# vkit-dev/vkit-ocr-model-adaptive-scaling

Measured on AMD Instinct MI355X. Metric: images/sec fwd+bwd @1024x1024 bf16 (train step: rough+precise passes, losses, backward, clip, AdamW), higher is better.
Workload: dtype bf16

## Files before the change

### include/vkas.h

```cpp
#ifndef VKAS_H
#define VKAS_H

#include <stddef.h>
#include <stdint.h>

#ifdef __cplusplus
extern "C" {
#endif

#define VKAS_F32 0
#define VKAS_BF16 1
#define VKAS_F16 2

#define VKAS_OK 0
#define VKAS_E_ARG (-1)
#define VKAS_E_LAUNCH (-2)

#define VKAS_EPI_NONE 0
#define VKAS_EPI_GELU 1
#define VKAS_EPI_SCALE_RES 2
#define VKAS_EPI_DGELU 3
#define VKAS_EPI_ADD 4
#define VKAS_EPI_PATCH 5
#define VKAS_EPI_HEAD 6
// ... 42 lines not shown
long vkas_layernorm_bwd_parts(long M, int Cp);
long vkas_scale_res_bwd_parts(long M, int Cp);
long vkas_dwconv7x7_wgrad_parts(int B, int H, int W, int Cp, int dtype);
int vkas_pad_vector(const float* v, float* out, int n, int np, void* stream);
size_t vkas_dw_weight_elems(int Cp);
int vkas_pack_dw_weight(const float* w, float* out, int C, int Cp, int flip, void* stream);
int vkas_unpack_dw_wgrad(const float* gw, float* grad, int C, int Cp, int accumulate, void* stream);
int vkas_image_nchw_to_nhwc8(const float* img, void* out, int B, int C, int H, int W, int dtype, void* stream);
int vkas_nhwc_to_nchw_f32(const void* x, long ld, float* out, int B, int H, int W, int C, int dtype, void* stream);
int vkas_nchw_f32_to_nhwc(const float* g, void* out, long ld, int B, int H, int W, int C, int Cp, int dtype, void* stream);

int vkas_conv_gemm_fwd(const void* x, const vkas_conv_geom* g, const void* Bw, int Np, const vkas_epilogue* epi,
                       int dtype, void* stream);
int vkas_conv_gemm_wgrad(const void* x, const vkas_conv_geom* g, const void* dy, long lddy, int Np, float* gw,
                         float* gb, int dtype, void* stream);
int vkas_conv_gemm_wgrad_ordered(const void* x, const vkas_conv_geom* g, const void* dy, long lddy, int Np, float* gw,
                                 int dtype, void* stream);
int vkas_conv_gemm_wgrad_gelu(const void* x, const vkas_conv_geom* g, const void* dy, long lddy, int Np, float* gw,
                              float* gb, int dtype, void* stream);

size_t vkas_upconv5_fold_elems(int Np, int Cp, int f, int transposed);
int vkas_upconv5_fold(const float* w, void* out, int N, int C, int Np, int Cp, int f, int transposed, int dtype, void* stream);
int vkas_upconv5_fwd(const void* x, const vkas_conv_geom* g, int f, const void* Bf, int Np, const float* bias, void* out,
                     long ldo, int dtype, void* stream);
int vkas_upconv5_dgrad(const void* dy, long lddy, const vkas_conv_geom* g, int f, const void* Bt, int Np, void* dx, long lddx,
                       int dtype, void* stream);
size_t vkas_upconv5_wgrad_ws_bytes(int B, int H, int W, int Np);
int vkas_upconv5_wgrad(const void* x, const vkas_conv_geom* g, int f, const void* dy, long lddy, int Np, void* ws,
                       size_t ws_bytes, float* gwf, float* gb, int dtype, void* stream);
int vkas_upconv5_unfold_wgrad(const float* gwf, float* dw, int N, int C, int Np, int Cp, int f, int accumulate, void* stream);

size_t vkas_mlp_chain_image_elems(int C);
int vkas_mlp_chain_pack(const float* w1, const float* w2, const float* b1, int C, int mode, void* img, int dtype,
                        void* stream);
int vkas_mlp_chain_fwd(const void* yn, long ldyn, const void* img, const float* b2, const void* x, long ldx,
                       const float* colscale, const float* rowscale, int rows_per_image, void* h, long ldh, void* z,
                       long ldz, void* out, long ldo, long M, int C, int dtype, void* stream);
int vkas_mlp_chain_ln_fwd(const void* y, long ldy, const float* ln_gamma, const float* ln_beta, void* yn, long ldyn,
                          float* stats, const void* img, const float* b2, const void* x, long ldx, const float* colscale,
                          const float* rowscale, int rows_per_image, void* h, long ldh, void* z, long ldz, void* out,
                          long ldo, long M, int C, int dtype, void* stream);
int vkas_mlp_chain_bwd(const void* dz, long lddz, const void* img_t, const void* h, long ldh, void* dh, long lddh,
                       void* dyn, long lddyn, long M, int C, int dtype, void* stream);
int vkas_conv_gemm_tile(int wgrad, long M, int Np, int K);
int vkas_conv_gemm_kernel_id(int wgrad, const vkas_conv_geom* g, int Np, long lddy, int head_width);
int vkas_colsum(const void* y, long ld, long M, int Np, float* out, int accumulate, float* ws, size_t ws_bytes,
                int dtype, void* stream);
size_t vkas_colsum_ws_bytes(long M, int Np);

int vkas_dwconv7x7_fwd(const void* x, long ldx, const float* w, const float* bias, const void* addend, long ldadd,
                       void* y, long ldy, int B, int H, int W, int Cp, int dtype, void* stream);
int vkas_dwconv7x7_wgrad(const void* x, long ldx, const void* dy, long lddy, float* gw, float* gb, float* ws,
                         size_t ws_bytes, int B, int H, int W, int Cp, int dtype, void* stream);
size_t vkas_dwconv7x7_wgrad_ws_bytes(int B, int H, int W, int Cp);

int vkas_layernorm_fwd(const void* x, long ldx, const float* gamma, const float* beta, void* y, long ldy,
                       float* stats, long M, int C, int Cp, int act_gelu, int dtype, void* stream);
int vkas_layernorm_bwd(const void* x, long ldx, const float* gamma, const float* beta, const float* stats,
                       const void* dy, long lddy, void* dx, long lddx, float* dgamma, float* dbeta, float* ws,
                       size_t ws_bytes, long M, int C, int Cp, int act_gelu, int dtype, void* stream);
size_t vkas_layernorm_bwd_ws_bytes(long M, int Cp);

int vkas_pack_head_params(const float* gamma, const float* beta, const float* wproj, const float* bproj, int C, int oc,
                          int pw, float* out, void* stream);
int vkas_head_tail_fwd(const void* z, long ldz, const vkas_head_desc* hd, long M, int dtype, void* stream);
int vkas_head_tail_bwd(const void* z, long ldz, const vkas_head_desc* hd, const float* const* dproj, void* dz, long lddz,
                       float* dparams, float* ws, size_t ws_bytes, long M, int dtype, void* stream);
size_t vkas_head_tail_bwd_ws_bytes(long M, int pw);

int vkas_scale_res_bwd(const void* dout, long lddo, const void* z, long ldz, const float* colscale,
                       const float* rowscale, int rows_per_image, void* dz, long lddz, float* dscale, float* dbias,
                       float* ws, size_t ws_bytes, long M, int Cp, int dtype, void* stream);
size_t vkas_scale_res_bwd_ws_bytes(long M, int Cp);

int vkas_resize_fwd(const void* x, long ldx, void* y, long ldy, int B, int Hin, int Win, int Hout, int Wout,
                    int Cp, int mode, int accumulate, int dtype, void* stream);
int vkas_resize_bwd(const void* dy, long lddy, void* dx, long lddx, int B, int Hin, int Win, int Hout, int Wout,
                    int Cp, int mode, int accumulate, int dtype, void* stream);
size_t vkas_resize_bwd_ws_bytes(int B, int Hin, int Win, int Hout, int Wout, int Cp);
int vkas_resize_bwd_ws(const void* dy, long lddy, void* dx, long lddx, float* ws, size_t ws_bytes, int B, int Hin, int Win,
                       int Hout, int Wout, int Cp, int mode, int accumulate, int dtype, void* stream);

int vkas_upconv_adj(const void* dz, long lddz, void* E, int B, int h, int w, int N, int dtype, void* stream);
int vkas_upconv_adj_unpack_wgrad(const float* gE, float* gwp, int N, int Cp, void* stream);

int vkas_adaptive_avgpool_fwd(const void* x, long ldx, void* y, long ldy, int B, int H, int W, int s, int Cp,
                              int dtype, void* stream);
int vkas_adaptive_avgpool_bwd(const void* dy, long lddy, void* dx, long lddx, int B, int H, int W, int s, int Cp,
                              int accumulate, int dtype, void* stream);

int vkas_copy_channels(const void* x, long ldx, void* y, long ldy, long M, int Cp, int accumulate, int dtype,
                       void* stream);
int vkas_copy_channel_range(const void* x, long ldx, int c_src, void* y, long ldy, int c_dst, long M, int C,
                            int zero_tail, int dtype, void* stream);
int vkas_softplus_fwd(const float* x, float* y, long n, void* stream);
int vkas_softplus_bwd(const float* x, const float* dy, float* dx, long n, void* stream);

typedef struct vkas_rough_loss_cfg {
  float focal_factor, dice_factor, l1_factor, score_min, height_min;
  float focal_alpha, focal_gamma;
  float out_scale;
} vkas_rough_loss_cfg;
int vkas_rough_loss_fwd(const float* mask_feat, const float* height_feat, const float* gt_mask,
                        const float* gt_score, int B, int H, int W, int up, int left, int CH, int CW,
                        const vkas_rough_loss_cfg* cfg, double* sums, float* loss, void* stream);
int vkas_rough_loss_bwd(const float* mask_feat, const float* height_feat, const float* gt_mask,
                        const float* gt_score, int B, int H, int W, int up, int left, int CH, int CW,
                        const vkas_rough_loss_cfg* cfg, const double* sums, const float* dloss, float* d_mask_feat,
                        float* d_height_feat, void* stream);

typedef struct vkas_precise_loss_cfg {
  float pos_l2, neg_l2, offset_l1, reg_l1, angle_ce, dist_l1, loss_factor;
  float smooth_beta;
  float out_scale;
} vkas_precise_loss_cfg;
int vkas_points_margin(const int64_t* py, const int64_t* px, long n, int H, int W, int64_t* margin, void* stream);
int vkas_precise_loss_fwd(const float* prob, const float* offset, const float* angle, const float* dist,
                          const float* gt_score, const float* gt_mask, const int64_t* py, const int64_t* px,
                          const float* gt_offsets, const float* gt_angles, const float* gt_dists, int B, int H,
                          int W, int up, int left, int CH, int CW, int P, const vkas_precise_loss_cfg* cfg,
                          double* sums, float* loss, void* stream);
int vkas_precise_loss_bwd(const float* prob, const float* offset, const float* angle, const float* dist,
                          const float* gt_score, const float* gt_mask, const int64_t* py, const int64_t* px,
                          const float* gt_offsets, const float* gt_angles, const float* gt_dists, int B, int H,
                          int W, int up, int left, int CH, int CW, int P, const vkas_precise_loss_cfg* cfg,
                          const double* sums, const float* dloss, float* d_prob, float* d_offset, float* d_angle,
                          float* d_dist, void* stream);
typedef struct vkas_precise_loss_extra_cfg {
  float mask_focal, prob_l1, prob_wahr;
  float prob_l1_beta;
  float wahr_gamma;
  float focal_alpha, focal_gamma;
} vkas_precise_loss_extra_cfg;
#define VKAS_PRECISE_LOSS_EX_SUMS 16
int vkas_precise_loss_ex_fwd(const float* prob, const float* offset, const float* angle, const float* dist,
                             const float* gt_score, const float* gt_mask, const int64_t* py, const int64_t* px,
                             const float* gt_offsets, const float* gt_angles, const float* gt_dists, int B, int H,
                             int W, int up, int left, int CH, int CW, int P, const vkas_precise_loss_cfg* cfg,
                             const float* mask_feat, const vkas_precise_loss_extra_cfg* ex, double* sums, float* loss,
                             void* stream);
int vkas_precise_loss_ex_bwd(const float* prob, const float* offset, const float* angle, const float* dist,
                             const float* gt_score, const float* gt_mask, const int64_t* py, const int64_t* px,
                             const float* gt_offsets, const float* gt_angles, const float* gt_dists, int B, int H,
                             int W, int up, int left, int CH, int CW, int P, const vkas_precise_loss_cfg* cfg,
                             const float* mask_feat, const vkas_precise_loss_extra_cfg* ex, const double* sums,
                             const float* dloss, float* d_prob, float* d_offset, float* d_angle, float* d_dist,
                             float* d_mask_feat, void* stream);

#define VKAS_LOSS_FOCAL 0
#define VKAS_LOSS_DICE 1
#define VKAS_LOSS_L1 2
#define VKAS_LOSS_SMOOTH_L1 3
#define VKAS_LOSS_L2 4
#define VKAS_LOSS_WAHR 5
int vkas_elementwise_loss_fwd(int kind, const float* pred, const float* gt, const float* mask, long n, float p0, float p1,
                              float eps, double* sums, float* loss, void* stream);
int vkas_elementwise_loss_bwd(int kind, const float* pred, const float* gt, const float* mask, long n, float p0, float p1,
                              float eps, const double* sums, const float* dloss, float* dpred, void* stream);
int vkas_cross_entropy_fwd(const float* logits, const void* target, int hard, long rows, int classes, double* sums,
                           float* loss, void* stream);
int vkas_cross_entropy_bwd(const float* logits, const void* target, int hard, long rows, int classes, const float* dloss,
                           float* dlogits, void* stream);

int vkas_points_prepare(const long* py, const long* px, int B, int P, int H, int W, int* map, int* pix, long Mp, void* stream);
int vkas_points_gather_rows(const void* z, long ldz, int c0, int Ns, const float* stats, const float* const* dproj,
                            int n_heads, long M, const int* pix, long Mp, void* zs, float* stats_s, float* dproj_s,
// ... 43 lines not shown
```

### vkit_ocr_model_adaptive_scaling_amd/_lib.py

```python
import ctypes
import os
from ctypes import POINTER, Structure, c_char_p, c_double, c_float, c_int, c_int64, c_long, c_longlong, c_size_t, c_void_p

_HERE = os.path.dirname(os.path.abspath(__file__))
LIB_PATH = os.environ.get('VKAS_LIB_PATH') or os.path.join(_HERE, 'libvkas.so')

F32, BF16, F16 = 0, 1, 2
EPI_NONE, EPI_GELU, EPI_SCALE_RES, EPI_DGELU, EPI_ADD, EPI_PATCH, EPI_HEAD = range(7)
LOSS_FOCAL, LOSS_DICE, LOSS_L1, LOSS_SMOOTH_L1, LOSS_L2 = range(5)
LOSS_WAHR = 5
PRECISE_LOSS_EX_SUMS = 16


class ConvGeom(Structure):
    _fields_ = [('B', c_int), ('Hin', c_int), ('Win', c_int), ('Hout', c_int), ('Wout', c_int), ('Cp', c_int),
                ('ldx', c_int), ('KH', c_int), ('KW', c_int), ('stride', c_int), ('pad', c_int)]


class HeadDesc(Structure):
    _fields_ = [('n_heads', c_int), ('pw', c_int), ('n0', c_int * 4), ('np', c_int * 4), ('c', c_int * 4),
                ('oc', c_int * 4), ('params', c_void_p), ('stats', c_void_p), ('proj', c_void_p)]


class Epilogue(Structure):
# ... 18 lines not shown
    _fields_ = [('pos_l2', c_float), ('neg_l2', c_float), ('offset_l1', c_float), ('reg_l1', c_float),
                ('angle_ce', c_float), ('dist_l1', c_float), ('loss_factor', c_float), ('smooth_beta', c_float),
                ('out_scale', c_float)]


class PreciseLossExtraCfg(Structure):
    _fields_ = [('mask_focal', c_float), ('prob_l1', c_float), ('prob_wahr', c_float), ('prob_l1_beta', c_float),
                ('wahr_gamma', c_float), ('focal_alpha', c_float), ('focal_gamma', c_float)]


class VkasError(RuntimeError):
    pass


if not os.path.exists(LIB_PATH):
    raise ImportError(
        f'{LIB_PATH} not found: build the HIP kernels first (python -c "import __graft_entry__ as g; g.build()" '
        f'or make -C {os.path.join(_HERE, "csrc")}).  There is no CPU fallback.')

lib = ctypes.CDLL(LIB_PATH)

_P = c_void_p
_SIGS = {
    'vkas_last_error': (c_char_p, []),
    'vkas_abi_version': (c_int, []),
    'vkas_pack_conv_weight': (c_int, [_P, _P, c_int, c_int, c_int, c_int, c_int, c_int, c_int, c_int, _P]),
    'vkas_pack_conv_weight_slice': (c_int, [_P, _P, c_int, c_int, c_int, c_int, c_int, c_int, c_int, c_int, c_int, c_int, _P]),
    'vkas_unpack_conv_wgrad': (c_int, [_P, _P, c_int, c_int, c_int, c_int, c_int, c_int, c_int, _P]),
    'vkas_accumulate_many': (c_int, [c_int, POINTER(c_void_p), POINTER(c_void_p), POINTER(c_int), _P]),
    'vkas_finalize_many': (c_int, [c_int, POINTER(c_void_p), POINTER(c_long), POINTER(c_int), POINTER(c_int), POINTER(c_void_p),
                                   POINTER(c_int), _P]),
    'vkas_layernorm_bwd_parts': (c_long, [c_long, c_int]),
    'vkas_scale_res_bwd_parts': (c_long, [c_long, c_int]),
    'vkas_dwconv7x7_wgrad_parts': (c_long, [c_int, c_int, c_int, c_int, c_int]),
    'vkas_pad_vector': (c_int, [_P, _P, c_int, c_int, _P]),
    'vkas_dw_weight_elems': (c_size_t, [c_int]),
    'vkas_pack_dw_weight': (c_int, [_P, _P, c_int, c_int, c_int, _P]),
    'vkas_unpack_dw_wgrad': (c_int, [_P, _P, c_int, c_int, c_int, _P]),
    'vkas_image_nchw_to_nhwc8': (c_int, [_P, _P, c_int, c_int, c_int, c_int, c_int, _P]),
    'vkas_nhwc_to_nchw_f32': (c_int, [_P, c_long, _P, c_int, c_int, c_int, c_int, c_int, _P]),
    'vkas_nchw_f32_to_nhwc': (c_int, [_P, _P, c_long, c_int, c_int, c_int, c_int, c_int, c_int, _P]),
    'vkas_conv_gemm_fwd': (c_int, [_P, POINTER(ConvGeom), _P, c_int, POINTER(Epilogue), c_int, _P]),
    'vkas_conv_gemm_wgrad': (c_int, [_P, POINTER(ConvGeom), _P, c_long, c_int, _P, _P, c_int, _P]),
    'vkas_conv_gemm_wgrad_ordered': (c_int, [_P, POINTER(ConvGeom), _P, c_long, c_int, _P, c_int, _P]),
    'vkas_conv_gemm_wgrad_gelu': (c_int, [_P, POINTER(ConvGeom), _P, c_long, c_int, _P, _P, c_int, _P]),
    'vkas_upconv5_fold_elems': (c_size_t, [c_int, c_int, c_int, c_int]),
    'vkas_upconv5_fold': (c_int, [_P, _P, c_int, c_int, c_int, c_int, c_int, c_int, c_int, _P]),
    'vkas_upconv5_fwd': (c_int, [_P, POINTER(ConvGeom), c_int, _P, c_int, _P, _P, c_long, c_int, _P]),
    'vkas_upconv5_dgrad': (c_int, [_P, c_long, POINTER(ConvGeom), c_int, _P, c_int, _P, c_long, c_int, _P]),
    'vkas_upconv5_wgrad_ws_bytes': (c_size_t, [c_int, c_int, c_int, c_int]),
    'vkas_upconv5_wgrad': (c_int, [_P, POINTER(ConvGeom), c_int, _P, c_long, c_int, _P, c_size_t, _P, _P, c_int, _P]),
    'vkas_upconv5_unfold_wgrad': (c_int, [_P, _P, c_int, c_int, c_int, c_int, c_int, c_int, _P]),
    'vkas_mlp_chain_image_elems': (c_size_t, [c_int]),
    'vkas_mlp_chain_pack': (c_int, [_P, _P, _P, c_int, c_int, _P, c_int, _P]),
    'vkas_mlp_chain_fwd': (c_int, [_P, c_long, _P, _P, _P, c_long, _P, _P, c_int, _P, c_long, _P, c_long, _P, c_long,
                                   c_long, c_int, c_int, _P]),
    'vkas_mlp_chain_ln_fwd': (c_int, [_P, c_long, _P, _P, _P, c_long, _P, _P, _P, _P, c_long, _P, _P, c_int, _P, c_long, _P,
                                      c_long, _P, c_long, c_long, c_int, c_int, _P]),
    'vkas_mlp_chain_bwd': (c_int, [_P, c_long, _P, _P, c_long, _P, c_long, _P, c_long, c_long, c_int, c_int, _P]),
    'vkas_conv_gemm_tile': (c_int, [c_int, c_long, c_int, c_int]),
    'vkas_conv_gemm_kernel_id': (c_int, [c_int, POINTER(ConvGeom), c_int, c_long, c_int]),
    'vkas_colsum': (c_int, [_P, c_long, c_long, c_int, _P, c_int, _P, c_size_t, c_int, _P]),
    'vkas_colsum_ws_bytes': (c_size_t, [c_long, c_int]),
    'vkas_dwconv7x7_fwd': (c_int, [_P, c_long, _P, _P, _P, c_long, _P, c_long, c_int, c_int, c_int, c_int, c_int, _P]),
    'vkas_dwconv7x7_wgrad': (c_int, [_P, c_long, _P, c_long, _P, _P, _P, c_size_t, c_int, c_int, c_int, c_int, c_int, _P]),
    'vkas_dwconv7x7_wgrad_ws_bytes': (c_size_t, [c_int, c_int, c_int, c_int]),
    'vkas_layernorm_fwd': (c_int, [_P, c_long, _P, _P, _P, c_long, _P, c_long, c_int, c_int, c_int, c_int, _P]),
    'vkas_layernorm_bwd': (c_int, [_P, c_long, _P, _P, _P, _P, c_long, _P, c_long, _P, _P, _P, c_size_t, c_long, c_int,
                                   c_int, c_int, c_int, _P]),
    'vkas_layernorm_bwd_ws_bytes': (c_size_t, [c_long, c_int]),
    'vkas_pack_head_params': (c_int, [_P, _P, _P, _P, c_int, c_int, c_int, _P, _P]),
    'vkas_head_tail_fwd': (c_int, [_P, c_long, _P, c_long, c_int, _P]),
    'vkas_head_tail_bwd': (c_int, [_P, c_long, POINTER(HeadDesc), POINTER(c_void_p), _P, c_long, _P, _P, c_size_t, c_long, c_int, _P]),
    'vkas_head_tail_bwd_ws_bytes': (c_size_t, [c_long, c_int]),
    'vkas_scale_res_bwd': (c_int, [_P, c_long, _P, c_long, _P, _P, c_int, _P, c_long, _P, _P, _P, c_size_t, c_long,
                                   c_int, c_int, _P]),
    'vkas_scale_res_bwd_ws_bytes': (c_size_t, [c_long, c_int]),
    'vkas_resize_fwd': (c_int, [_P, c_long, _P, c_long, c_int, c_int, c_int, c_int, c_int, c_int, c_int, c_int, c_int, _P]),
    'vkas_resize_bwd': (c_int, [_P, c_long, _P, c_long, c_int, c_int, c_int, c_int, c_int, c_int, c_int, c_int, c_int, _P]),
    'vkas_resize_bwd_ws_bytes': (c_size_t, [c_int, c_int, c_int, c_int, c_int, c_int]),
    'vkas_resize_bwd_ws': (c_int, [_P, c_long, _P, c_long, _P, c_size_t, c_int, c_int, c_int, c_int, c_int, c_int, c_int, c_int,
                                   c_int, _P]),
    'vkas_upconv_adj': (c_int, [_P, c_long, _P, c_int, c_int, c_int, c_int, c_int, _P]),
    'vkas_upconv_adj_unpack_wgrad': (c_int, [_P, _P, c_int, c_int, _P]),
    'vkas_adaptive_avgpool_fwd':(c_int, [_P, c_long, _P, c_long, c_int, c_int, c_int, c_int, c_int, c_int, _P]),
    'vkas_adaptive_avgpool_bwd': (c_int, [_P, c_long, _P, c_long, c_int, c_int, c_int, c_int, c_int, c_int, c_int, _P]),
    'vkas_copy_channels': (c_int, [_P, c_long, _P, c_long, c_long, c_int, c_int, c_int, _P]),
    'vkas_copy_channel_range': (c_int, [_P, c_long, c_int, _P, c_long, c_int, c_long, c_int, c_int, c_int, _P]),
    'vkas_softplus_fwd': (c_int, [_P, _P, c_long, _P]),
    'vkas_softplus_bwd': (c_int, [_P, _P, _P, c_long, _P]),
    'vkas_rough_loss_fwd': (c_int, [_P, _P, _P, _P, c_int, c_int, c_int, c_int, c_int, c_int, c_int,
                                    POINTER(RoughLossCfg), _P, _P, _P]),
    'vkas_rough_loss_bwd': (c_int, [_P, _P, _P, _P, c_int, c_int, c_int, c_int, c_int, c_int, c_int,
                                    POINTER(RoughLossCfg), _P, _P, _P, _P, _P]),
    'vkas_points_margin': (c_int, [_P, _P, c_long, c_int, c_int, _P, _P]),
    'vkas_precise_loss_fwd': (c_int, [_P] * 11 + [c_int] * 8 + [POINTER(PreciseLossCfg), _P, _P, _P]),
    'vkas_precise_loss_bwd': (c_int, [_P] * 11 + [c_int] * 8 + [POINTER(PreciseLossCfg), _P, _P, _P, _P, _P, _P, _P]),
    'vkas_precise_loss_ex_fwd': (c_int, [_P] * 11 + [c_int] * 8 + [POINTER(PreciseLossCfg), _P, POINTER(PreciseLossExtraCfg),
                                                                     _P, _P, _P]),
    'vkas_precise_loss_ex_bwd': (c_int, [_P] * 11 + [c_int] * 8 + [POINTER(PreciseLossCfg), _P, POINTER(PreciseLossExtraCfg)]
                                 + [_P] * 8),
    'vkas_elementwise_loss_fwd': (c_int, [c_int, _P, _P, _P, c_long, c_float, c_float, c_float, _P, _P, _P]),
    'vkas_elementwise_loss_bwd': (c_int, [c_int, _P, _P, _P, c_long, c_float, c_float, c_float, _P, _P, _P, _P]),
    'vkas_cross_entropy_fwd': (c_int, [_P, _P, c_int, c_long, c_int, _P, _P, _P]),
    'vkas_cross_entropy_bwd': (c_int, [_P, _P, c_int, c_long, c_int, _P, _P, _P]),
    'vkas_points_prepare': (c_int, [_P, _P, c_int, c_int, c_int, c_int, _P, _P, c_long, _P]),
    'vkas_points_gather_rows': (c_int, [_P, c_long, c_int, c_int, _P, _P, c_int, c_long, _P, c_long, _P, _P, _P, c_int, _P]),
    'vkas_points_gather_patches': (c_int, [_P, c_long, c_int, c_int, c_int, c_int, _P, c_long, _P, c_int, _P]),
    'vkas_points_scatter3x3': (c_int, [_P, _P, _P, c_long, c_int, c_int, c_int, c_int, _P, c_long, c_int, _P]),
    'vkas_points_scatter_vec8': (c_int, [_P, _P, c_long, _P, _P]),
    'vkas_points_gather_vec8': (c_int, [_P, _P, c_long, _P, _P]),
    'vkas_pack_many': (c_int, [_P, _P, c_int, c_int, _P]),
    'vkas_pack_many_blocks': (c_int, [_P]),
    'vkas_rough_postprocess': (c_int, [_P, _P, c_int, c_int, c_int, _P, _P, c_float, c_float, _P, _P, _P]),
    'vkas_precise_postprocess': (c_int, [_P, _P, _P, _P, c_int, c_int, c_int, _P, _P, _P, _P, _P, _P, _P]),
    'vkas_char_polygons_workspace_bytes': (c_long, [c_int, c_int, c_int, c_int]),
    'vkas_char_polygons': (c_int, [_P, _P, _P, _P, c_int, c_int, c_int, c_int, c_float, c_float, c_float, _P, c_size_t,
                                   _P, _P, _P, _P, _P]),
    'vkas_text_regions_workspace_bytes': (c_longlong, [c_int, c_int, c_int, c_int]),
    'vkas_text_regions': (c_int, [_P, _P, c_int, c_int, c_int, c_int, _P, c_longlong, _P, _P, _P, _P, _P, _P, _P]),
    'vkas_l2norm_sq': (c_int, [_P, c_long, _P, _P]),
    'vkas_adamw_step': (c_int, [_P, _P, _P, _P, c_long, _P, c_float, c_float, c_float, c_float, c_float, c_float,
                                c_float, c_int, _P]),
}

EXPORTS = tuple(_SIGS)

for _name, (_res, _args) in _SIGS.items():
    _fn = getattr(lib, _name)
    _fn.restype = _res
    _fn.argtypes = _args


def check(rc: int, what: str = ''):
    if rc != 0:
        msg = lib.vkas_last_error()
        raise VkasError(f'{what}: vkas error {rc}: {msg.decode() if msg else "?"}')
```

### vkit_ocr_model_adaptive_scaling_amd/csrc/upconv_adj.hip

```cpp
#include "vkas_common.h"

namespace {

__device__ __forceinline__ int xcd_row(unsigned bx, unsigned rows) {
  const unsigned xcd = bx & 7u, slot = bx >> 3;
  const unsigned q8 = rows >> 3, r8 = rows & 7u;
  return (int)((xcd < r8 ? xcd * (q8 + 1) : r8 * (q8 + 1) + (xcd - r8) * q8) + slot);
}

__device__ __forceinline__ void ut_weights(int i, int n, float* w) {
  w[0] = i == 0 ? 0.f : 0.25f;
  w[1] = i == 0 ? 1.f : 0.75f;
  w[2] = i == n - 1 ? 1.f : 0.75f;
  w[3] = i == n - 1 ? 0.f : 0.25f;
}

template <typename T>
__global__ __launch_bounds__(256) void upconv_adj_kernel(const T* __restrict__ dz, long lddz, T* __restrict__ E, int h,
                                                         int w, int nvec) {
  const int idx = blockIdx.y * 256 + threadIdx.x;
  const int j = idx / nvec;
  const int v = idx - j * nvec;
  if (j >= w) return;
  const int row = xcd_row(blockIdx.x, gridDim.x);
  const int b = row / h;
  const int i = row - b * h;
  const int H2 = 2 * h, W2 = 2 * w;
  float wy[4], wx[4];
  ut_weights(i, h, wy);
  ut_weights(j, w, wx);
  int xc[6];
  bool xok[6];
#pragma unroll
  for (int c = 0; c < 6; ++c) {
    const int X = 2 * j - 2 + c;
    xok[c] = X >= 0 && X < W2;
    xc[c] = X < 0 ? 0 : (X >= W2 ? W2 - 1 : X);
  }
  const T* db = dz + (long)b * H2 * W2 * lddz + v * 8;
  float acc[3][3][8];
#pragma unroll
  for (int ky = 0; ky < 3; ++ky)
#pragma unroll
    for (int kx = 0; kx < 3; ++kx)
#pragma unroll
      for (int k = 0; k < 8; ++k) acc[ky][kx][k] = 0.f;
#pragma unroll
  for (int r = 0; r < 6; ++r) {
    const int Y = 2 * i - 2 + r;
    const bool yok = Y >= 0 && Y < H2;
    const int yc = Y < 0 ? 0 : (Y >= H2 ? H2 - 1 : Y);
    const T* rowp = db + (long)yc * W2 * lddz;
    Raw8<T> raw[6];
#pragma unroll
    for (int c = 0; c < 6; ++c) raw[c].load(rowp + (long)xc[c] * lddz);
    float hs[3][8];
#pragma unroll
    for (int kx = 0; kx < 3; ++kx)
#pragma unroll
      for (int k = 0; k < 8; ++k) hs[kx][k] = 0.f;
#pragma unroll
    for (int c = 0; c < 6; ++c) {
      raw[c].keep_if(yok && xok[c]);
      float t[8];
      raw[c].unpack(t);
#pragma unroll
      for (int kx = 0; kx < 3; ++kx) {
        const int a = c - kx;
        if (a < 0 || a > 3) continue;
#pragma unroll
        for (int k = 0; k < 8; ++k) hs[kx][k] = fmaf(wx[a], t[k], hs[kx][k]);
      }
    }
#pragma unroll
    for (int ky = 0; ky < 3; ++ky) {
      const int a = r - ky;
      if (a < 0 || a > 3) continue;
#pragma unroll
      for (int kx = 0; kx < 3; ++kx)
#pragma unroll
        for (int k = 0; k < 8; ++k) acc[ky][kx][k] = fmaf(wy[a], hs[kx][k], acc[ky][kx][k]);
    }
  }
  const long N = (long)nvec * 8;
  T* dst = E + (((long)b * h + i) * w + j) * (9 * N) + v * 8;
#pragma unroll
  for (int ky = 0; ky < 3; ++ky)
#pragma unroll
    for (int kx = 0; kx < 3; ++kx) store8(dst + (ky * 3 + kx) * N, acc[ky][kx]);
}

__global__ __launch_bounds__(256) void upconv_adj_unpack_kernel(const float* __restrict__ gE, float* __restrict__ gwp, int N,
                                                                int Cp4, long total4) {
  for (long i = (long)blockIdx.x * 256 + threadIdx.x; i < total4; i += (long)gridDim.x * 256) {
    const int c4 = (int)(i % Cp4);
    const long r = i / Cp4;
    const int n = (int)(r % N);
    const int k = (int)(r / N);
    const float4 s = reinterpret_cast<const float4*>(gE)[i];
    float4* d = reinterpret_cast<float4*>(gwp) + ((long)n * 9 + (8 - k)) * Cp4 + c4;
    float4 o = *d;
    o.x += s.x; o.y += s.y; o.z += s.z; o.w += s.w;
    *d = o;
  }
}

}

extern "C" int vkas_upconv_adj(const void* dz, long lddz, void* E, int B, int h, int w, int N, int dtype, void* stream) {
  VKAS_CHECK(dz && E && vkas_aligned16(dz) && vkas_aligned16(E), "vkas_upconv_adj: null/misaligned tensor");
  VKAS_CHECK(B >= 0 && h > 0 && w > 0, "vkas_upconv_adj: bad spatial dims");
  VKAS_CHECK(N > 0 && N % 8 == 0 && lddz >= N && lddz % 8 == 0, "vkas_upconv_adj: bad channels/stride (N=%d lddz=%ld)", N, lddz);
  VKAS_CHECK(dtype == VKAS_BF16 || dtype == VKAS_F16, "vkas_upconv_adj: 16-bit storage only");
  if (B == 0) return VKAS_OK;
  VKAS_CHECK((long)B * h < (1L << 31) && (long)w * (N / 8) < (1L << 30) && vkas_cdiv((long)w * (N / 8), 256) <= 65535,
             "vkas_upconv_adj: map too large");
  dim3 grid((unsigned)((long)B * h), (unsigned)vkas_cdiv((long)w * (N / 8), 256));
  if (dtype == VKAS_BF16)
    upconv_adj_kernel<bf16_t><<<grid, 256, 0, vkas_stream(stream)>>>((const bf16_t*)dz, lddz, (bf16_t*)E, h, w, N / 8);
  else
    upconv_adj_kernel<f16_t><<<grid, 256, 0, vkas_stream(stream)>>>((const f16_t*)dz, lddz, (f16_t*)E, h, w, N / 8);
  VKAS_LAUNCH_CHECK("upconv_adj");
  return VKAS_OK;
}

extern "C" int vkas_upconv_adj_unpack_wgrad(const float* gE, float* gwp, int N, int Cp, void* stream) {
  VKAS_CHECK(gE && gwp && vkas_aligned16(gE) && vkas_aligned16(gwp), "vkas_upconv_adj_unpack_wgrad: null/misaligned pointer");
  VKAS_CHECK(N > 0 && Cp > 0 && Cp % 8 == 0, "vkas_upconv_adj_unpack_wgrad: bad sizes (N=%d Cp=%d)", N, Cp);
  const long total4 = 9L * N * (Cp / 4);
  long g = vkas_cdiv(total4, 256);
  if (g > 4096) g = 4096;
  upconv_adj_unpack_kernel<<<(unsigned)g, 256, 0, vkas_stream(stream)>>>(gE, gwp, N, Cp / 4, total4);
  VKAS_LAUNCH_CHECK("upconv_adj_unpack_wgrad");
  return VKAS_OK;
}
```

### vkit_ocr_model_adaptive_scaling_amd/ops.py

```python
import ctypes
import os
import weakref
from typing import Optional, Sequence, Tuple

import torch
from torch.autograd import Function

from . import _lib
from ._lib import lib, check, ConvGeom, Epilogue

_FLOAT = torch.float32


def rup8(c: int) -> int:
    return (c + 7) // 8 * 8


_DTYPE_CODES = {torch.float32: _lib.F32, torch.bfloat16: _lib.BF16, torch.float16: _lib.F16}
_MFMA_DTYPES = (torch.bfloat16, torch.float16)


def _dtc(dtype: torch.dtype) -> int:
    try:
        return _DTYPE_CODES[dtype]
# ... 914 lines not shown
        geom = _geom(B, H, W, H, W, Cp, act_ld(x), 3, 3, 1, 1)
        Bw = pack_head_weights(ws, nps, Cp, 0, x.dtype)
        if in_epilogue:
            conv_gemm(x, geom, Bw, Nt, z, _lib.EPI_HEAD, bias=b_cat, nk=(sum(cs), C * 9), head=head)
        else:
            conv_gemm(x, geom, Bw, Nt, z, _lib.EPI_NONE, bias=b_cat, nk=(sum(cs), C * 9))
            check(lib.vkas_head_tail_fwd(_p(z), Nt, ctypes.byref(head), M, _dt(x), _stream()), 'head_tail_fwd')
        if keep:
            ctx.save_for_backward(x, z, stats, hp, *ws, *bs, *gammas, *betas, *wps, *bps, *(() if x_low is None else (x_low,)))
        ctx.meta = (cs, ocs, nps, pw, C)
        ctx.low = x_low is not None
        return tuple(proj[h] for h in range(n_heads))

    @staticmethod
    def backward(ctx, *dprojs):
        cs, ocs, nps, pw, C = ctx.meta
        n_heads = len(cs)
        saved = ctx.saved_tensors
        x, z, stats, hp = saved[:4]
        ws, bs = saved[4:4 + n_heads], saved[4 + n_heads:4 + 2 * n_heads]
        B, H, W, Cp = x.shape
        Nt = z.shape[3]
        M = B * H * W
        K = 9 * Cp
        dev = x.device
        PS = 6 * pw + 8
        offs = [sum(nps[:h]) for h in range(n_heads + 1)]
        dparams = torch.empty((n_heads, PS), dtype=_FLOAT, device=dev)
        flat_sinks = all(grad_sink(p) is not None for p in list(ws) + list(bs))
        gbuf = zeros_f32(Nt * K + Nt, dev, flat_sinks)
        gwp, gbp = gbuf[:Nt * K], gbuf[Nt * K:]
        dps = []
        for h in range(n_heads):
            dp = dprojs[h]
            dps.append(torch.zeros((B, H, W, 8), dtype=_FLOAT, device=dev) if dp is None else dp.contiguous().float())

        def tail_bwd(h0, h1, z_ptr, ldz, stats_ptr, dp_ptrs, rows, dz):
            head = _lib.HeadDesc()
            head.n_heads, head.pw = h1 - h0, pw
            ptrs = (ctypes.c_void_p * 4)()
            for j, h in enumerate(range(h0, h1)):
                head.n0[j], head.np[j], head.c[j], head.oc[j] = offs[h] - offs[h0], nps[h], cs[h], ocs[h]
                ptrs[j] = dp_ptrs[j]
            head.params, head.stats, head.proj = hp.data_ptr() + h0 * PS * 4, stats_ptr, None
            nbytes = lib.vkas_head_tail_bwd_ws_bytes(rows, pw)
            ws_buf = _ws(nbytes, dev)
            width = offs[h1] - offs[h0]
            _timed('head_tail_bwd_kernel', x, 0.0, rows, width, 0,
                   lambda: check(lib.vkas_head_tail_bwd(ctypes.c_void_p(z_ptr), ldz, ctypes.byref(head), ptrs, _p(dz), width,
                                                        ctypes.c_void_p(dparams.data_ptr() + h0 * PS * 4), _p(ws_buf), nbytes,
                                                        rows, _dt(x), _stream()), 'head_tail_bwd'),
                   float(rows) * (2 * width * x.element_size() + (h1 - h0) * 40))

        sp = _point_sparse_run(dprojs, B, H, W) if _POINT_SPARSE else None
        d0, d1 = (0, n_heads) if sp is None else ((0, sp[0]) if sp[0] > 0 else (sp[1], n_heads))
        es = x.element_size()
        low = ctx.low
        x_low = saved[4 + 6 * n_heads] if low else None
        h_, w_ = H // 2, W // 2
        need_dx = ctx.needs_input_grad[0]
        dx = (new_act(B, h_, w_, Cp, x) if low else new_act(B, H, W, Cp, x)) if need_dx else None

        def dense_dz(r0, r1):
            dz = new_act(B, H, W, offs[r1] - offs[r0], x)
            tail_bwd(r0, r1, z.data_ptr() + offs[r0] * es, Nt, stats.data_ptr() + r0 * M * 8,
                     [dps[h].data_ptr() for h in range(r0, r1)], M, dz)
            return dz

        def dense_upres(r0, r1, dx_up):
            Nd = offs[r1] - offs[r0]
            dz = dense_dz(r0, r1)
            geom = _geom(B, H, W, H, W, Cp, act_ld(x), 3, 3, 1, 1)
            conv_wgrad(x, geom, dz, Nd, nk=(sum(cs[r0:r1]), C * 9), with_bias=True,
                       gw_into=gwp[offs[r0] * K:offs[r1] * K], gb_into=gbp[offs[r0]:offs[r1]])
            if dx_up is not None:
                Bt = pack_head_weights(ws[r0:r1], nps[r0:r1], Cp, 1, x.dtype)
                g2 = _geom(B, H, W, H, W, Nd, Nd, 3, 3, 1, 1)
                conv_gemm(dz, g2, Bt, Cp, dx_up, _lib.EPI_NONE, nk=(C, sum(cs[r0:r1]) * 9))

        def dense_lowres(r0, r1):
            Nd = offs[r1] - offs[r0]
            dz = dense_dz(r0, r1)
            E = new_act(B, h_, w_, 9 * Nd, x)
            _timed('upconv_adj_kernel', x, 0.0, M // 4, 9 * Nd, 0,
                   lambda: check(lib.vkas_upconv_adj(_p(dz), act_ld(dz), _p(E), B, h_, w_, Nd, _dt(x), _stream()), 'upconv_adj'),
                   float(M) * Nd * es * 3.25)
            nbytes = lib.vkas_colsum_ws_bytes(M, Nd)
            ws_cs = _ws(nbytes, dev)
            _timed('colsum_partial_kernel', x, 0.0, M, Nd, 0,
                   lambda: check(lib.vkas_colsum(_p(dz), act_ld(dz), M, Nd, _p(gbp[offs[r0]:offs[r1]]), 1, _p(ws_cs), nbytes,
                                                 _dt(x), _stream()), 'colsum'), float(M) * Nd * es)
            del dz
            g1 = _geom(B, h_, w_, h_, w_, Cp, act_ld(x_low), 1, 1, 1, 0)
            gE = conv_wgrad(x_low, g1, E, 9 * Nd, nk=(9 * sum(cs[r0:r1]), C), step_scratch=True)
            check(lib.vkas_upconv_adj_unpack_wgrad(_p(gE), _p(gwp[offs[r0] * K:offs[r1] * K]), Nd, Cp, _stream()),
                  'upconv_adj_unpack_wgrad')
            if dx is not None:
                Bt = pack_head_weights(ws[r0:r1], nps[r0:r1], Cp, 1, x.dtype)
                g2 = _geom(B, h_, w_, h_, w_, 9 * Nd, 9 * Nd, 1, 1, 1, 0)
                conv_gemm(E, g2, Bt, Cp, dx, _lib.EPI_NONE, nk=(C, sum(cs[r0:r1]) * 9))

        dx_pts = dx
        dx_low_set = False
        if not low:
            if d1 > d0:
                dense_upres(d0, d1, dx)
            elif dx is not None:
                dx.zero_()
        else:
            marked = [point_mark(dprojs[h]) is not None for h in range(d0, d1)]
            plain = [d0 + i for i, m in enumerate(marked) if not m]
            e0, e1 = (plain[0], plain[-1] + 1) if plain else (d0, d0)
            if plain != list(range(e0, e1)) or (e0 > d0 and e1 < d1):
                e0, e1 = d0, d0
            u0, u1 = (e1, d1) if e0 == d0 else (d0, e0)
            dx_pts = None
            if u1 > u0:
                dx_pts = new_act(B, H, W, Cp, x) if need_dx else None
                dense_upres(u0, u1, dx_pts)
            elif sp is not None and need_dx:
                dx_pts = torch.zeros((B, H, W, Cp), dtype=x.dtype, device=dev)
            if e1 > e0:
                dense_lowres(e0, e1)
                dx_low_set = True
        if sp is not None:
            s0, s1, py, px = sp
            Ns = offs[s1] - offs[s0]
            P = py.shape[1]
            Mp = -(-(B * P) // 64) * 64
            scratch = torch.empty((M + Mp,), dtype=torch.int32, device=dev)
            pmap, pix = scratch[:M], scratch[M:]
            check(lib.vkas_points_prepare(_p(py), _p(px), B, P, H, W, _p(pmap), _p(pix), Mp, _stream()), 'points_prepare')
            zs = new_act(1, 1, Mp, Ns, x)
            fbuf = torch.empty(((s1 - s0) * Mp * 10,), dtype=_FLOAT, device=dev)
            stats_s, dproj_s = fbuf[:(s1 - s0) * Mp * 2], fbuf[(s1 - s0) * Mp * 2:]
            ptrs = (ctypes.c_void_p * 4)(*[dps[h].data_ptr() for h in range(s0, s1)])
            check(lib.vkas_points_gather_rows(_p(z), Nt, offs[s0], Ns, ctypes.c_void_p(stats.data_ptr() + s0 * M * 8), ptrs,
                                              s1 - s0, M, _p(pix), Mp, _p(zs), _p(stats_s), _p(dproj_s), _dt(x), _stream()),
                  'points_gather_rows')
            dzs = new_act(1, 1, Mp, Ns, x)
            tail_bwd(s0, s1, zs.data_ptr(), Ns, stats_s.data_ptr(),
                     [dproj_s.data_ptr() + j * Mp * 32 for j in range(s1 - s0)], Mp, dzs)
            xs = new_act(1, 1, Mp, K, x)
            check(lib.vkas_points_gather_patches(_p(x), act_ld(x), Cp, B, H, W, _p(pix), Mp, _p(xs), _dt(x), _stream()),
                  'points_gather_patches')
            g1 = _geom(1, 1, Mp, 1, Mp, K, K, 1, 1, 1, 0)
            conv_wgrad(xs, g1, dzs, Ns, nk=(sum(cs[s0:s1]), C * 9), with_bias=True,
                       gw_into=gwp[offs[s0] * K:offs[s1] * K], gb_into=gbp[offs[s0]:offs[s1]])
            if dx is not None:
                Wf = pack_head_weights(ws, nps, Cp, 0, x.dtype)[offs[s0] * K:offs[s1] * K].view(1, 1, Ns, K)
                dzt = dzs.view(Mp, Ns).t().contiguous().view(1, 1, Ns, Mp)
                g3 = _geom(1, 1, Ns, 1, Ns, K, K, 1, 1, 1, 0)
                D = conv_wgrad(Wf, g3, dzt, Mp, nk=(B * P, C * 9), step_scratch=True, ordered=True)
                check(lib.vkas_points_scatter3x3(_p(D), _p(pix), _p(pmap), Mp, B, H, W, Cp, _p(dx_pts), act_ld(dx_pts), _dt(x),
                                                 _stream()), 'points_scatter3x3')
        if low and dx is not None:
            if dx_pts is not None:
                _timed('resize2x_bwd_kernel', x, 0.0, M, Cp, 0,
                       lambda: check(lib.vkas_resize_bwd(_p(dx_pts), act_ld(dx_pts), _p(dx), act_ld(dx), B, h_, w_, H, W, Cp, 0,
                                                         int(dx_low_set), _dt(x), _stream()), 'resize_bwd'),
                       B * Cp * es * (h_ * w_ * (2 if dx_low_set else 1) + H * W))
            elif not dx_low_set:
                dx.zero_()
        gws, gbs = [], []
        for h in range(n_heads):
            gslice = gwp[offs[h] * K:offs[h + 1] * K]
            sw = grad_sink(ws[h])
            if sw is not None:
                unpack_wgrad(gslice, (cs[h], C, 3, 3), nps[h], Cp, into=ws[h].grad)
                sw[0].grad_delivered(sw[1])
                gws.append(None)
            else:
                gws.append(unpack_wgrad(gslice, (cs[h], C, 3, 3), nps[h], Cp))
            gbs.append(gbp[offs[h]:offs[h] + cs[h]])
# ... 974 lines not shown
```

Before: 277.4.

## Fuse bias column-sum into upconv adjoint kernel and narrow its vector width

The low-resolution dense head backward no longer runs a separate colsum pass over dz. The upconv adjoint kernel now also accumulates per-block partial sums of the centre taps, which cover each dz pixel exactly once. An optional compact kernel then reduces those partials, and the result is finalized into the bias gradient. The default vector width also drops from 8 to 4 channels per thread with higher occupancy bounds; in exchange there are more blocks, a shared-memory reduction and an extra compact launch.

```diff
diff --git a/include/vkas.h b/include/vkas.h
--- a/include/vkas.h
+++ b/include/vkas.h
@@ -148,6 +148,10 @@
                        int Hout, int Wout, int Cp, int mode, int accumulate, int dtype, void* stream);
 
 int vkas_upconv_adj(const void* dz, long lddz, void* E, int B, int h, int w, int N, int dtype, void* stream);
+size_t vkas_upconv_adj_ws_bytes(int B, int h, int w, int N);
+long vkas_upconv_adj_parts(int B, int h, int w, int N);
+int vkas_upconv_adj_ws(const void* dz, long lddz, void* E, int B, int h, int w, int N, float* ws, size_t ws_bytes, int dtype,
+                       void* stream);
 int vkas_upconv_adj_unpack_wgrad(const float* gE, float* gwp, int N, int Cp, void* stream);
 
 int vkas_adaptive_avgpool_fwd(const void* x, long ldx, void* y, long ldy, int B, int H, int W, int s, int Cp,
diff --git a/vkit_ocr_model_adaptive_scaling_amd/_lib.py b/vkit_ocr_model_adaptive_scaling_amd/_lib.py
--- a/vkit_ocr_model_adaptive_scaling_amd/_lib.py
+++ b/vkit_ocr_model_adaptive_scaling_amd/_lib.py
@@ -124,6 +124,9 @@
     'vkas_resize_bwd_ws': (c_int, [_P, c_long, _P, c_long, _P, c_size_t, c_int, c_int, c_int, c_int, c_int, c_int, c_int, c_int,
                                    c_int, _P]),
     'vkas_upconv_adj': (c_int, [_P, c_long, _P, c_int, c_int, c_int, c_int, c_int, _P]),
+    'vkas_upconv_adj_ws': (c_int, [_P, c_long, _P, c_int, c_int, c_int, c_int, _P, c_size_t, c_int, _P]),
+    'vkas_upconv_adj_ws_bytes': (c_size_t, [c_int, c_int, c_int, c_int]),
+    'vkas_upconv_adj_parts': (c_long, [c_int, c_int, c_int, c_int]),
     'vkas_upconv_adj_unpack_wgrad': (c_int, [_P, _P, c_int, c_int, _P]),
     'vkas_adaptive_avgpool_fwd':(c_int, [_P, c_long, _P, c_long, c_int, c_int, c_int, c_int, c_int, c_int, _P]),
     'vkas_adaptive_avgpool_bwd': (c_int, [_P, c_long, _P, c_long, c_int, c_int, c_int, c_int, c_int, c_int, c_int, _P]),
diff --git a/vkit_ocr_model_adaptive_scaling_amd/csrc/upconv_adj.hip b/vkit_ocr_model_adaptive_scaling_amd/csrc/upconv_adj.hip
--- a/vkit_ocr_model_adaptive_scaling_amd/csrc/upconv_adj.hip
+++ b/vkit_ocr_model_adaptive_scaling_amd/csrc/upconv_adj.hip
@@ -15,13 +15,32 @@
   w[3] = i == n - 1 ? 0.f : 0.25f;
 }
 
-template <typename T>
-__global__ __launch_bounds__(256) void upconv_adj_kernel(const T* __restrict__ dz, long lddz, T* __restrict__ E, int h,
-                                                         int w, int nvec) {
+template <typename T, int V> struct RawV;
+template <typename T> struct RawV<T, 8> : Raw8<T> {};
+template <> struct RawV<bf16_t, 4> {
+  bf16x4 a;
+  __device__ __forceinline__ void load(const bf16_t* p) { a = *reinterpret_cast<const bf16x4*>(p); }
+  __device__ __forceinline__ void keep_if(bool k) { if (!k) for (int i = 0; i < 4; ++i) a[i] = (bf16_t)0.f; }
+  __device__ __forceinline__ void unpack(float* v) const { for (int i = 0; i < 4; ++i) v[i] = (float)a[i]; }
+};
+template <> struct RawV<f16_t, 4> {
+  f16x4 a;
+  __device__ __forceinline__ void load(const f16_t* p) { a = *reinterpret_cast<const f16x4*>(p); }
+  __device__ __forceinline__ void keep_if(bool k) { if (!k) for (int i = 0; i < 4; ++i) a[i] = (f16_t)0.f; }
+  __device__ __forceinline__ void unpack(float* v) const { for (int i = 0; i < 4; ++i) v[i] = (float)a[i]; }
+};
+template <typename T> __device__ __forceinline__ void storeV(T* p, const float (&v)[8]) { store8(p, v); }
+template <typename T> __device__ __forceinline__ void storeV(T* p, const float (&v)[4]) { store4(p, v); }
+
+template <typename T, int V, bool SUMS>
+__global__ __launch_bounds__(256, V == 4 ? 4 : 1) void upconv_adj_kernel(const T* __restrict__ dz, long lddz, T* __restrict__ E, int h,
+                                                         int w, int nvec, float* __restrict__ part) {
   const int idx = blockIdx.y * 256 + threadIdx.x;
-  const int j = idx / nvec;
-  const int v = idx - j * nvec;
-  if (j >= w) return;
+  const int j0 = idx / nvec;
+  const int v = idx - j0 * nvec;
+  const bool live = j0 < w;
+  if (!SUMS && !live) return;
+  const int j = live ? j0 : w - 1;
   const int row = xcd_row(blockIdx.x, gridDim.x);
   const int b = row / h;
   const int i = row - b * h;
@@ -37,39 +56,46 @@
     xok[c] = X >= 0 && X < W2;
     xc[c] = X < 0 ? 0 : (X >= W2 ? W2 - 1 : X);
   }
-  const T* db = dz + (long)b * H2 * W2 * lddz + v * 8;
-  float acc[3][3][8];
+  const T* db = dz + (long)b * H2 * W2 * lddz + v * V;
+  float acc[3][3][V];
+  float bs[V];
+#pragma unroll
+  for (int k = 0; k < V; ++k) bs[k] = 0.f;
 #pragma unroll
   for (int ky = 0; ky < 3; ++ky)
 #pragma unroll
     for (int kx = 0; kx < 3; ++kx)
 #pragma unroll
-      for (int k = 0; k < 8; ++k) acc[ky][kx][k] = 0.f;
+      for (int k = 0; k < V; ++k) acc[ky][kx][k] = 0.f;
 #pragma unroll
   for (int r = 0; r < 6; ++r) {
     const int Y = 2 * i - 2 + r;
     const bool yok = Y >= 0 && Y < H2;
     const int yc = Y < 0 ? 0 : (Y >= H2 ? H2 - 1 : Y);
     const T* rowp = db + (long)yc * W2 * lddz;
-    Raw8<T> raw[6];
+    RawV<T, V> raw[6];
 #pragma unroll
     for (int c = 0; c < 6; ++c) raw[c].load(rowp + (long)xc[c] * lddz);
-    float hs[3][8];
+    float hs[3][V];
 #pragma unroll
     for (int kx = 0; kx < 3; ++kx)
 #pragma unroll
-      for (int k = 0; k < 8; ++k) hs[kx][k] = 0.f;
+      for (int k = 0; k < V; ++k) hs[kx][k] = 0.f;
 #pragma unroll
     for (int c = 0; c < 6; ++c) {
       raw[c].keep_if(yok && xok[c]);
-      float t[8];
+      float t[V];
       raw[c].unpack(t);
+      if (SUMS && (r == 2 || r == 3) && (c == 2 || c == 3)) {
+#pragma unroll
+        for (int k = 0; k < V; ++k) bs[k] += t[k];
+      }
 #pragma unroll
       for (int kx = 0; kx < 3; ++kx) {
         const int a = c - kx;
         if (a < 0 || a > 3) continue;
 #pragma unroll
-        for (int k = 0; k < 8; ++k) hs[kx][k] = fmaf(wx[a], t[k], hs[kx][k]);
+        for (int k = 0; k < V; ++k) hs[kx][k] = fmaf(wx[a], t[k], hs[kx][k]);
       }
     }
 #pragma unroll
@@ -79,15 +105,50 @@
 #pragma unroll
       for (int kx = 0; kx < 3; ++kx)
 #pragma unroll
-        for (int k = 0; k < 8; ++k) acc[ky][kx][k] = fmaf(wy[a], hs[kx][k], acc[ky][kx][k]);
-    }
-  }
-  const long N = (long)nvec * 8;
-  T* dst = E + (((long)b * h + i) * w + j) * (9 * N) + v * 8;
-#pragma unroll
-  for (int ky = 0; ky < 3; ++ky)
-#pragma unroll
-    for (int kx = 0; kx < 3; ++kx) store8(dst + (ky * 3 + kx) * N, acc[ky][kx]);
+        for (int k = 0; k < V; ++k) acc[ky][kx][k] = fmaf(wy[a], hs[kx][k], acc[ky][kx][k]);
+    }
+  }
+  const long N = (long)nvec * V;
+  if (live) {
+    T* dst = E + (((long)b * h + i) * w + j) * (9 * N) + v * V;
+#pragma unroll
+    for (int ky = 0; ky < 3; ++ky)
+#pragma unroll
+      for (int kx = 0; kx < 3; ++kx) storeV(dst + (ky * 3 + kx) * N, acc[ky][kx]);
+  }
+  if constexpr (SUMS) {
+    __shared__ float red[256 * V];
+#pragma unroll
+    for (int k = 0; k < V; ++k) red[threadIdx.x * V + k] = live ? bs[k] : 0.f;
+    __syncthreads();
+    const int first = (int)(((long)blockIdx.y * 256) % nvec);
+    float* prow = part + ((long)blockIdx.x * gridDim.y + blockIdx.y) * N;
+    for (int n = threadIdx.x; n < (int)N; n += 256) {
+      const int vv = n / V, k = n - vv * V;
+      int t = vv - first;
+      if (t < 0) t += nvec;
+      float s = 0.f;
+      for (; t < 256; t += nvec) s += red[t * V + k];
+      prow[n] = s;
+    }
+  }
+}
+
+constexpr long UPADJ_PARTS = 1024;
+__global__ __launch_bounds__(256) void upconv_adj_compact_kernel(const float* __restrict__ fine, long R, long rpb, int N,
+                                                                 float* __restrict__ out) {
+  const long r0 = (long)blockIdx.x * rpb;
+  const long r1 = r0 + rpb < R ? r0 + rpb : R;
+  for (int n = threadIdx.x; n < N; n += 256) {
+    float s[4] = {0.f, 0.f, 0.f, 0.f};
+    long r = r0;
+    for (; r + 3 < r1; r += 4) {
+#pragma unroll
+      for (int q = 0; q < 4; ++q) s[q] += fine[(r + q) * N + n];
+    }
+    for (; r < r1; ++r) s[0] += fine[r * N + n];
+    out[(long)blockIdx.x * N + n] = (s[0] + s[1]) + (s[2] + s[3]);
+  }
 }
 
 __global__ __launch_bounds__(256) void upconv_adj_unpack_kernel(const float* __restrict__ gE, float* __restrict__ gwp, int N,
@@ -107,21 +168,66 @@
 
 }
 
-extern "C" int vkas_upconv_adj(const void* dz, long lddz, void* E, int B, int h, int w, int N, int dtype, void* stream) {
+namespace {
+int upadj_vec() {
+  static const int vec = (getenv("VKAS_UPADJ_VEC") && atoi(getenv("VKAS_UPADJ_VEC")) == 8) ? 8 : 4;
+  return vec;
+}
+long upadj_fine_rows(int B, int h, int w, int N) { return (long)B * h * vkas_cdiv((long)w * (N / upadj_vec()), 256); }
+
+template <typename T, int V>
+void upadj_launch(dim3 grid, const void* dz, long lddz, void* E, int h, int w, int N, float* part, hipStream_t st) {
+  if (part) upconv_adj_kernel<T, V, true><<<grid, 256, 0, st>>>((const T*)dz, lddz, (T*)E, h, w, N / V, part);
+  else upconv_adj_kernel<T, V, false><<<grid, 256, 0, st>>>((const T*)dz, lddz, (T*)E, h, w, N / V, nullptr);
+}
+}
+
+extern "C" long vkas_upconv_adj_parts(int B, int h, int w, int N) {
+  if (B <= 0 || h <= 0 || w <= 0 || N <= 0) return 0;
+  const long R = upadj_fine_rows(B, h, w, N);
+  return R <= UPADJ_PARTS ? R : vkas_cdiv(R, vkas_cdiv(R, UPADJ_PARTS));
+}
+
+extern "C" size_t vkas_upconv_adj_ws_bytes(int B, int h, int w, int N) {
+  if (B <= 0 || h <= 0 || w <= 0 || N <= 0) return 0;
+  const long R = upadj_fine_rows(B, h, w, N);
+  return (size_t)(R <= UPADJ_PARTS ? R : R + vkas_upconv_adj_parts(B, h, w, N)) * (size_t)N * sizeof(float);
+}
+
+extern "C" int vkas_upconv_adj_ws(const void* dz, long lddz, void* E, int B, int h, int w, int N, float* ws, size_t ws_bytes,
+                                  int dtype, void* stream) {
   VKAS_CHECK(dz && E && vkas_aligned16(dz) && vkas_aligned16(E), "vkas_upconv_adj: null/misaligned tensor");
   VKAS_CHECK(B >= 0 && h > 0 && w > 0, "vkas_upconv_adj: bad spatial dims");
   VKAS_CHECK(N > 0 && N % 8 == 0 && lddz >= N && lddz % 8 == 0, "vkas_upconv_adj: bad channels/stride (N=%d lddz=%ld)", N, lddz);
   VKAS_CHECK(dtype == VKAS_BF16 || dtype == VKAS_F16, "vkas_upconv_adj: 16-bit storage only");
   if (B == 0) return VKAS_OK;
-  VKAS_CHECK((long)B * h < (1L << 31) && (long)w * (N / 8) < (1L << 30) && vkas_cdiv((long)w * (N / 8), 256) <= 65535,
+  const int V = upadj_vec();
+  VKAS_CHECK((long)B * h < (1L << 31) && (long)w * (N / V) < (1L << 30) && vkas_cdiv((long)w * (N / V), 256) <= 65535,
              "vkas_upconv_adj: map too large");
-  dim3 grid((unsigned)((long)B * h), (unsigned)vkas_cdiv((long)w * (N / 8), 256));
-  if (dtype == VKAS_BF16)
-    upconv_adj_kernel<bf16_t><<<grid, 256, 0, vkas_stream(stream)>>>((const bf16_t*)dz, lddz, (bf16_t*)E, h, w, N / 8);
-  else
-    upconv_adj_kernel<f16_t><<<grid, 256, 0, vkas_stream(stream)>>>((const f16_t*)dz, lddz, (f16_t*)E, h, w, N / 8);
+  VKAS_CHECK(!ws || (vkas_aligned16(ws) && ws_bytes >= vkas_upconv_adj_ws_bytes(B, h, w, N)),
+             "vkas_upconv_adj: workspace misaligned or too small");
+  hipStream_t st = vkas_stream(stream);
+  dim3 grid((unsigned)((long)B * h), (unsigned)vkas_cdiv((long)w * (N / V), 256));
+  const long R = (long)grid.x * grid.y;
+  const long P = vkas_upconv_adj_parts(B, h, w, N);
+  float* fine = ws ? (R <= UPADJ_PARTS ? ws : ws + P * N) : nullptr;
+  if (dtype == VKAS_BF16) {
+    if (V == 8) upadj_launch<bf16_t, 8>(grid, dz, lddz, E, h, w, N, fine, st);
+    else upadj_launch<bf16_t, 4>(grid, dz, lddz, E, h, w, N, fine, st);
+  } else {
+    if (V == 8) upadj_launch<f16_t, 8>(grid, dz, lddz, E, h, w, N, fine, st);
+    else upadj_launch<f16_t, 4>(grid, dz, lddz, E, h, w, N, fine, st);
+  }
   VKAS_LAUNCH_CHECK("upconv_adj");
+  if (ws && R > UPADJ_PARTS) {
+    upconv_adj_compact_kernel<<<(unsigned)P, 256, 0, st>>>(fine, R, vkas_cdiv(R, UPADJ_PARTS), N, ws);
+    VKAS_LAUNCH_CHECK("upconv_adj_compact");
+  }
   return VKAS_OK;
+}
+
+extern "C" int vkas_upconv_adj(const void* dz, long lddz, void* E, int B, int h, int w, int N, int dtype, void* stream) {
+  return vkas_upconv_adj_ws(dz, lddz, E, B, h, w, N, nullptr, 0, dtype, stream);
 }
 
 extern "C" int vkas_upconv_adj_unpack_wgrad(const float* gE, float* gwp, int N, int Cp, void* stream) {
diff --git a/vkit_ocr_model_adaptive_scaling_amd/ops.py b/vkit_ocr_model_adaptive_scaling_amd/ops.py
--- a/vkit_ocr_model_adaptive_scaling_amd/ops.py
+++ b/vkit_ocr_model_adaptive_scaling_amd/ops.py
@@ -1020,14 +1020,12 @@
             Nd = offs[r1] - offs[r0]
             dz = dense_dz(r0, r1)
             E = new_act(B, h_, w_, 9 * Nd, x)
+            nbytes = lib.vkas_upconv_adj_ws_bytes(B, h_, w_, Nd)
+            ws_cs = _ws(nbytes, dev)
             _timed('upconv_adj_kernel', x, 0.0, M // 4, 9 * Nd, 0,
-                   lambda: check(lib.vkas_upconv_adj(_p(dz), act_ld(dz), _p(E), B, h_, w_, Nd, _dt(x), _stream()), 'upconv_adj'),
-                   float(M) * Nd * es * 3.25)
-            nbytes = lib.vkas_colsum_ws_bytes(M, Nd)
-            ws_cs = _ws(nbytes, dev)
-            _timed('colsum_partial_kernel', x, 0.0, M, Nd, 0,
-                   lambda: check(lib.vkas_colsum(_p(dz), act_ld(dz), M, Nd, _p(gbp[offs[r0]:offs[r1]]), 1, _p(ws_cs), nbytes,
-                                                 _dt(x), _stream()), 'colsum'), float(M) * Nd * es)
+                   lambda: check(lib.vkas_upconv_adj_ws(_p(dz), act_ld(dz), _p(E), B, h_, w_, Nd, _p(ws_cs), nbytes, _dt(x),
+                                                        _stream()), 'upconv_adj'), float(M) * Nd * es * 3.25)
+            finalize_many([(ws_cs, 0, lib.vkas_upconv_adj_parts(B, h_, w_, Nd), Nd, Nd, gbp[offs[r0]:offs[r1]], True)])
             del dz
             g1 = _geom(B, h_, w_, h_, w_, Cp, act_ld(x_low), 1, 1, 1, 0)
             gE = conv_wgrad(x_low, g1, E, 9 * Nd, nk=(9 * sum(cs[r0:r1]), C), step_scratch=True)
```

Measured after the change: 276.4. No clear change (-0.3%).
